# gitAugust/Aruco_Slam

Hardware: AMD Instinct MI355X
Metric: frames/s (detect+pose+EKF) at 1280x720, 20 markers, 200 landmarks (higher is better)
Workload: dtype u8/f64; 1 GPU; cfg2: 1280x720 gray stream per GPU, 20 markers/frame in view, 200-landmark EKF (N=603), frames resident in HBM, detector {'polygonalApproxAccuracyRate': 0.03, 'doCornerRefinement': 1}; streams=1, ekf=True, asserted=every frame: 20 markers detected, 20 corrections fused, map_gather=none

## Files before the change

aruco_slam_amd/csrc/detect.hip:

```cpp
#include "common.h"
#include "detect.h"
#include <cfloat>
#include <climits>
#include <cstdlib>
#include <algorithm>

namespace aslam {

__device__ __forceinline__ int dir_dx(int s) { return (int)((0x901Au >> (2 * s)) & 3u) - 1; }
__device__ __forceinline__ int dir_dy(int s) { return (int)((0xA901u >> (2 * s)) & 3u) - 1; }
__device__ __forceinline__ int first_outer(unsigned m) { return (m & 1u) ? 0 : (m & 128u) ? 7 : (m & 64u) ? 6 : 5; }
__device__ __forceinline__ int first_hole(unsigned m) { return 31 - __clz((int)(m & 0xFEu)); }


__device__ __forceinline__ unsigned byte_is_zero(unsigned x) { return ~(((x & 0x7F7F7F7Fu) + 0x7F7F7F7Fu) | x) & 0x80808080u; }

constexpr int TW = 64, TH = 32, HALO = 12;
constexpr int LW = TW + 2 * HALO;
constexpr int LH = TH + 2 * HALO;
constexpr int kBlockStarts = 1024;

template <int R> __device__ __forceinline__ bool box_is_fg(const unsigned (*I)[LW + 1], int ly, int lx, int v_plus_c) {
    constexpr int k2 = (2 * R + 1) * (2 * R + 1);
    const int sum = (int)(I[ly + R + 1][lx + R + 1] - I[ly - R][lx + R + 1] - I[ly + R + 1][lx - R] + I[ly - R][lx - R]);
    return 2 * sum >= k2 * (2 * v_plus_c - 1);
}
__device__ __forceinline__ bool box_is_fg_r(const unsigned (*I)[LW + 1], int ly, int lx, int R, int v_plus_c) {
    const int k2 = (2 * R + 1) * (2 * R + 1);
    const int sum = (int)(I[ly + R + 1][lx + R + 1] - I[ly - R][lx + R + 1] - I[ly + R + 1][lx - R] + I[ly - R][lx - R]);
    return 2 * sum >= k2 * (2 * v_plus_c - 1);
}

#ifdef ASLAM_THR_STAMPS
#define THR_STAMP(i) do { if (tid == 0 && blockIdx.x == 4000) tst[i] = clock64(); } while (0)
#else
#define THR_STAMP(i) do { } while (0)
#endif
template <bool kDefaultWindows>
__global__ __launch_bounds__(256) void k_threshold(const uint8_t* __restrict__ in, int channels, size_t in_frame_stride,
                                                   size_t in_row_step, uint8_t* __restrict__ gray_out,
                                                   uint8_t* __restrict__ nbr, DetectCfg cfg,
                                                   unsigned* __restrict__ starts, unsigned* __restrict__ n_starts,
                                                   unsigned* __restrict__ nodeplane, Counters* ctr, int nframes) {
    __shared__ uint8_t g[LH][LW + 4];
    __shared__ unsigned I[LH + 1][LW + 1];
    __shared__ unsigned long long sRow[kScales][TH + 2];
    __shared__ unsigned long long sRing[kScales][2];
    __shared__ unsigned sLutRow[3][64];
    __shared__ unsigned sStart[kBlockStarts];
    __shared__ unsigned sNStart, sBase;

    const int tid = threadIdx.x;
    const int rows = cfg.rows, cols = cfg.cols;
    const unsigned gx = (unsigned)(cols + TW - 1) / TW, gy = (unsigned)(rows + TH - 1) / TH;
    const unsigned per_xcd = gridDim.x >> 3;
    const unsigned logical = (blockIdx.x & 7u) * per_xcd + (blockIdx.x >> 3);
    if (logical >= gx * gy * (unsigned)nframes) return;
    const int b = (int)(logical / (gx * gy));
    const unsigned rem = logical - (unsigned)b * gx * gy;
    const int x0 = (int)(rem % gx) * TW, y0 = (int)(rem / gx) * TH;
    const uint8_t* src = in + (size_t)b * in_frame_stride;
#ifdef ASLAM_THR_STAMPS
    long long tst[8] = {0};
#endif
    if (tid == 0) sNStart = 0;
    THR_STAMP(0);

    if (channels == 1 && (in_row_step & 3) == 0 && ((size_t)src & 3) == 0) {
        constexpr int kPasses = (LH * (LW / 4) + 255) / 256;
        unsigned v[kPasses];
#pragma unroll
        for (int p = 0; p < kPasses; p++) {
            const int i = tid + 256 * p;
            v[p] = 0;
            if (i < LH * (LW / 4)) {
                const int ly = i / (LW / 4), q = i - ly * (LW / 4);
                const int gy = min(max(y0 + ly - HALO, 0), rows - 1);
                const int gx = x0 + 4 * q - HALO;
                const uint8_t* rowp = src + (size_t)gy * in_row_step;
                if (gx >= 0 && gx + 3 < cols) {
                    v[p] = *reinterpret_cast<const unsigned*>(rowp + gx);
                } else {
                    for (int k = 0; k < 4; k++) v[p] |= (unsigned)rowp[min(max(gx + k, 0), cols - 1)] << (8 * k);
                }
            }
        }
#pragma unroll
        for (int p = 0; p < kPasses; p++) {
            const int i = tid + 256 * p;
            if (i < LH * (LW / 4)) {
                const int ly = i / (LW / 4), q = i - ly * (LW / 4);
                *reinterpret_cast<unsigned*>(&g[ly][4 * q]) = v[p];
            }
        }
    } else {
        for (int i = tid; i < LH * LW; i += 256) {
            int ly = i / LW, lx = i - ly * LW;
            int gx = min(max(x0 + lx - HALO, 0), cols - 1);
            int gy = min(max(y0 + ly - HALO, 0), rows - 1);
            const uint8_t* p = src + (size_t)gy * in_row_step + (size_t)gx * channels;
            unsigned v;
            if (channels == 3) v = (p[0] * 1868u + p[1] * 9617u + p[2] * 4899u + 8192u) >> 14;
            else v = p[0];
            g[ly][lx] = (uint8_t)v;
        }
    }
    __syncthreads();
    THR_STAMP(1);

    if (gray_out != nullptr) {
        for (int i = tid; i < TH * TW; i += 256) {
            int ty = i / TW, tx = i - ty * TW;
            int gx = x0 + tx, gy = y0 + ty;
            if (gx < cols && gy < rows) gray_out[((size_t)b * rows + gy) * cols + gx] = g[ty + HALO][tx + HALO];
        }
    }

    {
        const int q = tid >> 6, r = tid & 63;
        if (r < LH) {
            unsigned s = 0;
            for (int k = 0; k < LW / 4; k++) { s += g[r][q * (LW / 4) + k]; I[r + 1][q * (LW / 4) + k + 1] = s; }
        }
        if (tid < LW + 1) I[0][tid] = 0;
        if (tid < LH) I[tid + 1][0] = 0;
        __syncthreads();
        unsigned add = 0;
        if (r < LH)
            for (int qq = 0; qq < q; qq++) add += I[r + 1][(qq + 1) * (LW / 4)];
        __syncthreads();
        if (r < LH && q > 0)
            for (int k = 0; k < LW / 4; k++) I[r + 1][q * (LW / 4) + k + 1] += add;
    }
    __syncthreads();
    {
        const int h = tid >> 7, c = tid & 127;
        if (c < LW) {
            unsigned s = 0;
            for (int k = 0; k < LH / 2; k++) { s += I[h * (LH / 2) + k + 1][c + 1]; I[h * (LH / 2) + k + 1][c + 1] = s; }
        }
        __syncthreads();
        if (c < LW && h == 1) {
            const unsigned add = I[LH / 2][c + 1];
            for (int k = 0; k < LH / 2; k++) I[LH / 2 + k + 1][c + 1] += add;
        }
    }
    __syncthreads();
    THR_STAMP(2);

    auto thr_bits = [&](int by, int bx) -> unsigned {
        const int gx = x0 + bx - 1, gy = y0 + by - 1;
        unsigned bits = 0;
        if (gx >= 0 && gx < cols && gy >= 0 && gy < rows) {
            const int lx = bx - 1 + HALO, ly = by - 1 + HALO;
            const int vc = (int)g[ly][lx] + cfg.thresh_c;
            if (kDefaultWindows) {
                if (box_is_fg<1>(I, ly, lx, vc)) bits |= 1u;
                if (box_is_fg<6>(I, ly, lx, vc)) bits |= 2u;
                if (box_is_fg<11>(I, ly, lx, vc)) bits |= 4u;
            } else {
#pragma unroll
                for (int s = 0; s < kScales; s++)
                    if (s < cfg.n_scales && box_is_fg_r(I, ly, lx, cfg.win_r[s], vc)) bits |= 1u << s;
            }
        }
        return bits;
    };
    {
        const int wave = tid >> 6, lane = tid & 63;
        for (int by = wave; by < TH + 2; by += 4) {
            const unsigned bits = thr_bits(by, lane);
#pragma unroll
            for (int s = 0; s < kScales; s++) {
                const unsigned long long row = __ballot((bits >> s) & 1u);
                if (lane == 0) sRow[s][by] = row;
            }
        }
        if (wave < 2) {
            const unsigned bits = lane < TH + 2 ? thr_bits(lane, TW + wave) : 0u;
#pragma unroll
            for (int s = 0; s < kScales; s++) {
                const unsigned long long col = __ballot((bits >> s) & 1u);
                if (lane == 0) sRing[s][wave] = col;
            }
        }
        if (tid < 3 * 64) {
            const unsigned r = tid >> 6, v = tid & 63u;
            unsigned w = 0;
            for (unsigned j = 0; j < 4; j++) {
                const unsigned a = (v >> j) & 1u, b = (v >> (j + 1)) & 1u, c = (v >> (j + 2)) & 1u;
                const unsigned m = r == 0 ? (c << 1) | (b << 2) | (a << 3) : r == 1 ? c | (a << 4) : (a << 5) | (b << 6) | (c << 7);
                w |= m << (8 * j);
            }
            sLutRow[r][v] = w;
        }
    }
    __syncthreads();
    THR_STAMP(3);

    for (int u = tid; u < TH * TW / 4; u += 256) {
        const int ty = u / (TW / 4), tx4 = (u - ty * (TW / 4)) * 4;
        const int gy = y0 + ty;
        const bool row_on_grid = (gy & cfg.cut_mask) == 0;
        const unsigned grid4 = row_on_grid ? 15u : ((tx4 & cfg.cut_mask) == 0 ? 1u : 0u);
        unsigned out[kScales] = {0, 0, 0};
        unsigned emit = 0;
#pragma unroll
        for (int s = 0; s < kScales; s++) {
            unsigned six[3];
#pragma unroll
            for (int r = 0; r < 3; r++) {
                const int by = ty + r;
                unsigned v = (unsigned)(sRow[s][by] >> tx4) & 63u;
                if (tx4 == TW - 4) v |= ((unsigned)(sRing[s][0] >> by) & 1u) << 4 | ((unsigned)(sRing[s][1] >> by) & 1u) << 5;
                six[r] = v;
            }
            const unsigned m4 = sLutRow[0][six[0]] | sLutRow[1][six[1]] | sLutRow[2][six[2]];
            out[s] = m4;
            const unsigned fgb = (((six[1] >> 1) & 15u) * 0x00204081u & 0x01010101u) << 7;
            const unsigned hole_x = (m4 & 0x03030303u) ^ 0x02020202u;
            const unsigned cand = fgb & ((byte_is_zero(m4 & 0x1E1E1E1Eu) & ~byte_is_zero(m4)) | byte_is_zero(hole_x));
            emit |= (((cand >> 7) | (cand >> 14) | (cand >> 21) | (cand >> 28)) & 15u) << (4 * s);
            emit |= (((six[1] >> 1) & grid4) & 15u) << (4 * s);
        }
        for (unsigned rest = emit; rest; rest &= rest - 1u) {
            const int bit = __ffs((int)rest) - 1, s = bit >> 2, j = bit & 3;
            const unsigned gx = (unsigned)(x0 + tx4 + j);
            const unsigned m = (out[s] >> (8 * j)) & 0xFFu;
            const bool outer = m != 0 && (m & 0x1Eu) == 0, hole = (m & 3u) == 2u;
            const unsigned s0 = outer ? (unsigned)first_outer(m) : (unsigned)first_hole(m);
            unsigned cut = 0;
            if (row_on_grid || (gx & (unsigned)cfg.cut_mask) == 0) cut = m & ~((m >> 1) | (m << 7)) & 0xFFu;
            if (outer || hole) cut &= ~(1u << s0);
            const unsigned cnt = (unsigned)__popc(cut) + ((outer || hole) ? 1u : 0u);
            if (cnt == 0) continue;
            const unsigned k = atomicAdd(&sNStart, cnt);
            const bool staged = k + cnt <= (unsigned)kBlockStarts;
            unsigned kk = 0;
            bool fits = true;
            if (!staged) {
                for (unsigned e = k; e < (unsigned)kBlockStarts; e++) sStart[e] = kNone;
                kk = atomicAdd(&n_starts[b], cnt);
                fits = kk + cnt <= cfg.cap_starts;
                if (fits) nodeplane[((size_t)b * kScales + s) * nbr_plane_bytes(rows, cfg.pitch) + nbr_index((int)gx, gy, cfg.pitch)] = kk;
                else atomicOr(&ctr->overflow, (unsigned)kOvfStarts);
            }
            unsigned e = 0;
            auto put = [&](unsigned v) {
                if (staged) sStart[k + e] = v;
                else if (fits) starts[(size_t)b * cfg.cap_starts + kk + e] = v;
                e++;
            };
            if (outer || hole) put(pack_node(gx, (unsigned)gy, s0, (unsigned)s, outer ? kNodeOuter : kNodeHole));
            for (unsigned c2 = cut; c2; c2 &= c2 - 1u) put(pack_node(gx, (unsigned)gy, (unsigned)(__ffs((int)c2) - 1), (unsigned)s, kNodeCut));
        }
        if (gy < rows) {
#pragma unroll
            for (int s = 0; s < kScales; s++) {
                unsigned* dst = reinterpret_cast<unsigned*>(nbr + ((size_t)b * kScales + s) * nbr_plane_bytes(rows, cfg.pitch) +
                                                            nbr_index(x0 + tx4, gy, cfg.pitch));
                *dst = out[s];
            }
        }
    }
    __syncthreads();
    THR_STAMP(4);
    const unsigned ns = min(sNStart, (unsigned)kBlockStarts);
    if (tid == 0 && ns > 0) sBase = atomicAdd(&n_starts[b], ns);
    __syncthreads();
    for (unsigned i = tid; i < ns; i += 256) {
        const unsigned k = sBase + i, e = sStart[i];
        if (k < cfg.cap_starts) {
            starts[(size_t)b * cfg.cap_starts + k] = e;
            if (e != kNone && (i == 0 || ((sStart[i - 1] ^ e) & kNodePixelMask) != 0))
                nodeplane[((size_t)b * kScales + ((e >> 27) & 3u)) * nbr_plane_bytes(rows, cfg.pitch) +
                          nbr_index((int)(e & 0xFFFu), (int)((e >> 12) & 0xFFFu), cfg.pitch)] = k;
        } else {
            atomicOr(&ctr->overflow, (unsigned)kOvfStarts);
        }
    }
#ifdef ASLAM_THR_STAMPS
    THR_STAMP(5);
    if (tid == 0 && blockIdx.x == 4000) printf("thr tile: load %lld integral %lld threshold %lld masks %lld flush %lld\n", tst[1] - tst[0], tst[2] - tst[1], tst[3] - tst[2], tst[4] - tst[3], tst[5] - tst[4]);
#endif
}

__global__ __launch_bounds__(256) void k_clear_counts(int nframes, Counters* ctr, unsigned* a0, unsigned* a1, unsigned* a2, unsigned* a3, unsigned* a4) {
    const int i = blockIdx.x * 256 + threadIdx.x;
    if (i < kCounterHeads) reinterpret_cast<unsigned*>(ctr)[i] = 0u;
    if (i < nframes) { a0[i] = 0u; a1[i] = 0u; a2[i] = 0u; a3[i] = 0u; a4[i] = 0u; }
}

__global__ __launch_bounds__(256) void k_prefix(int nframes, const unsigned* __restrict__ counts, unsigned cap, unsigned per_ticket,
                                                unsigned* __restrict__ pre ) {
    __shared__ unsigned sPart[256];
    const int tid = threadIdx.x;
    const int per = (nframes + 255) / 256;
    unsigned s = 0;
    for (int k = 0; k < per; k++) {
        int f = tid * per + k;
        if (f < nframes) s += (min(counts[f], cap) + per_ticket - 1) / per_ticket;
    }
    sPart[tid] = s;
    __syncthreads();
    if (tid == 0) {
        unsigned acc = 0;
        for (int i = 0; i < 256; i++) { unsigned v = sPart[i]; sPart[i] = acc; acc += v; }
        pre[nframes] = acc;
    }
    __syncthreads();
    unsigned acc = sPart[tid];
    for (int k = 0; k < per; k++) {
        int f = tid * per + k;
        if (f < nframes) { pre[f] = acc; acc += (min(counts[f], cap) + per_ticket - 1) / per_ticket; }
    }
}

__device__ __forceinline__ int ticket_frame(const unsigned* sPre, int nframes, unsigned ticket) {
    int lo = 0, hi = nframes;
    while (hi - lo > 1) {
        int mid = (lo + hi) >> 1;
        if (sPre[mid] <= ticket) lo = mid; else hi = mid;
    }
    return lo;
}

constexpr int kMaxFramesPerCall = 1024;

__device__ __forceinline__ void load_ticket_ranges(unsigned* sPre, const unsigned* __restrict__ pre, const unsigned* __restrict__ counts,
                                                   unsigned cap, int nframes, int tid, int nthreads) {
    if (nframes == 1) {
        if (tid == 0) { sPre[0] = 0u; sPre[1] = min(counts[0], cap); }
    } else {
        for (int i = tid; i <= nframes; i += nthreads) sPre[i] = pre[i];
    }
}

struct Walk {
    int x, y, s;
};
__device__ __forceinline__ void walk_step(Walk& w, unsigned m) {
    unsigned r = ((m | (m << 8)) >> (w.s + 1)) & 0xFFu;
    int k = __ffs((int)r) - 1;
    int s2 = (w.s + 1 + k) & 7;
    w.x += dir_dx(s2);
    w.y += dir_dy(s2);
    w.s = (s2 + 4) & 7;
}

constexpr int kTraceChunk = 64;
constexpr int kSegRepsBusy = 32, kSegRepsRefill = 8;


__device__ __forceinline__ void build_step_table(unsigned short* sStep, int tid, int nthreads) {
    for (int i = tid; i < 256 * 8; i += nthreads) {
        const unsigned m = (unsigned)i >> 3;
        const int sd = i & 7;
        Walk t{0, 0, sd};
        if (m != 0) walk_step(t, m);
        const bool co = m != 0 && (m & 0x1Eu) == 0 && sd == first_outer(m);
        const bool ch = (m & 3u) == 2u && sd == first_hole(m);
        const bool cut = ((m >> sd) & 1u) != 0 && ((m >> ((sd + 1) & 7)) & 1u) == 0;
        sStep[i] = (unsigned short)((unsigned)(t.x + 1) | ((unsigned)(t.y + 1) << 2) | ((unsigned)t.s << 4) | (co ? 0x80u : 0u) | (ch ? 0x100u : 0u) |
                                    (cut ? 0x200u : 0u));
    }
}
__device__ __forceinline__ bool on_cut_grid(int x, int y, int mask) { return ((x & mask) == 0) || ((y & mask) == 0); }

__global__ __launch_bounds__(64) void k_seg(const uint8_t* __restrict__ nbr, DetectCfg cfg, int nframes,
                                            const unsigned* __restrict__ starts, const unsigned* __restrict__ n_starts,
                                            const unsigned* __restrict__ nodeplane,
                                            const unsigned* __restrict__ pre, Counters* ctr,
                                            NodeRec* __restrict__ nodes) {
    __shared__ unsigned sPre[kMaxFramesPerCall + 1];
    __shared__ unsigned short sStep[256 * 8];
    const int lane = threadIdx.x & 63;
    build_step_table(sStep, lane, 64);
    load_ticket_ranges(sPre, pre, n_starts, cfg.cap_starts, nframes, lane, 64);
    __syncthreads();
    const unsigned total = sPre[nframes];
    const int pitch = cfg.pitch;
    const size_t plane_bytes = nbr_plane_bytes(cfg.rows, pitch);

    int mode = 0;
    bool drained = false;
    unsigned lo = 0, hi = 0;
    const uint8_t* plane = nbr;
    const unsigned* idplane = nodeplane;
    Walk w{0, 0, 0};
    int n = 0, f = 0, area = 0;
    unsigned self = 0, state0 = 0;

    for (;;) {
        const unsigned long long idle = __ballot(mode == 0);
        if (idle != 0ull && !drained) {
            if (lo == hi) {
                unsigned base = 0;
                if (lane == 0) base = atomicAdd(&ctr->q_trace, (unsigned)kTraceChunk);
                base = __shfl(base, 0);
                lo = base;
                hi = min(base + (unsigned)kTraceChunk, total);
                if (lo >= total) { drained = true; lo = hi = 0; }
            }
            const unsigned take = min((unsigned)__popcll(idle), hi - lo);
            const unsigned rank = (unsigned)__popcll(idle & ((1ull << lane) - 1ull));
            if (mode == 0 && rank < take) {
                const unsigned ticket = lo + rank;
                if (!(ticket >= sPre[f] && ticket < sPre[f + 1])) f = ticket_frame(sPre, nframes, ticket);
                self = ticket - sPre[f];
                const unsigned e = starts[(size_t)f * cfg.cap_starts + self];
                const unsigned type = (e >> 29) & 3u;
                if (type == kNodeInvalid) {
                    nodes[(size_t)f * cfg.cap_starts + self] = NodeRec{kNone, kNone, 0u, 0};
                } else {
                    const int x = (int)(e & 0xFFFu), y = (int)((e >> 12) & 0xFFFu);
                    const unsigned sc = (e >> 27) & 3u;
                    plane = nbr + ((size_t)f * kScales + sc) * plane_bytes;
                    idplane = nodeplane + ((size_t)f * kScales + sc) * plane_bytes;
                    state0 = e;
                    w = Walk{x, y, (int)((e >> 24) & 7u)};
                    area = 0;
                    n = 0;
                    mode = 1;
                }
            }
            lo += take;
        }
        if (__ballot(mode != 0) == 0ull) {
            if (drained) break;
            continue;
        }
        const int reps = (idle == 0ull || drained) ? kSegRepsBusy : kSegRepsRefill;
        for (int rep = 0; rep < reps; rep++) {
            if (mode == 1) {
                const unsigned m = plane[nbr_index(w.x, w.y, pitch)];
                const unsigned st = sStep[(m << 3) | (unsigned)w.s];
                const bool arrived = n > 0 && ((st & 0x180u) != 0 || ((st & 0x200u) != 0 && on_cut_grid(w.x, w.y, cfg.cut_mask)));
                if (arrived) {
                    const unsigned want = pack_node((unsigned)w.x, (unsigned)w.y, (unsigned)w.s, (state0 >> 27) & 3u, 0u);
                    const unsigned cnt = min(n_starts[f], cfg.cap_starts);
                    unsigned id = idplane[nbr_index(w.x, w.y, pitch)];
                    unsigned found = kNone;
                    for (int t = 0; t < 9 && id < cnt; t++, id++) {
                        const unsigned e2 = starts[(size_t)f * cfg.cap_starts + id];
                        if (((e2 ^ want) & kNodePixelMask) != 0) break;
                        if (((e2 ^ want) & kNodeStateMask) == 0) { found = id; break; }
                    }
                    nodes[(size_t)f * cfg.cap_starts + self] = NodeRec{state0, found, (unsigned)n, area};
                    mode = 0;
                } else {
                    const int ddx = (int)(st & 3u) - 1, ddy = (int)((st >> 2) & 3u) - 1;
                    area += w.x * ddy - ddx * w.y;
                    w.x += ddx; w.y += ddy; w.s = (int)((st >> 4) & 7u);
                    n++;
                    if (n > cfg.max_perim) {
                        nodes[(size_t)f * cfg.cap_starts + self] = NodeRec{state0, kNone, (unsigned)n, area};
                            mode = 0;
                    }
                }
            }
            if (__ballot(mode != 0) == 0ull) break;
        }
    }
}

__device__ __forceinline__ int node_key(unsigned state, int cols) {
    return (int)((state >> 12) & 0xFFFu) * cols + (int)(state & 0xFFFu) + (((state >> 29) & 3u) == kNodeHole ? 1 : 0);
}
__device__ __forceinline__ void void_tickets(WriteRec* wl, unsigned wbase, unsigned wcap, unsigned cap_write) {
    for (unsigned long long t = wbase; t < (unsigned long long)wbase + wcap && t < cap_write; t++) wl[t] = WriteRec{0u, kNone, 0u, 0u};
}
constexpr int kLinkThreads = 1024;
constexpr unsigned kLinkLdsNodes = 32000;
constexpr unsigned kLinkSlots = 1536;
struct LinkSlot {
    int a;
    int b;
    int c;
    unsigned d;
};
__global__ __launch_bounds__(kLinkThreads) void k_link(DetectCfg cfg, const unsigned* __restrict__ n_starts, Counters* ctr,
                                                       const NodeRec* __restrict__ nodes, unsigned lds_nodes, unsigned* __restrict__ link_todo,
                                                       ContourRec* __restrict__ contours, unsigned* __restrict__ n_contours,
                                                       unsigned* __restrict__ n_points, WriteRec* __restrict__ wlist, unsigned* __restrict__ n_write) {
    ASLAM_DYN_LDS(dyn_lds);
    __shared__ unsigned sNSlots, sActive;
    const int tid = threadIdx.x;
    const int f = blockIdx.x;
    const int cols = cfg.cols;
    const unsigned nn = min(n_starts[f], cfg.cap_starts);
    const NodeRec* gn = nodes + (size_t)f * cfg.cap_starts;
    if (nn > lds_nodes) {
        if (tid == 0) link_todo[f] = 1u;
        return;
    }
    unsigned* sPair = reinterpret_cast<unsigned*>(dyn_lds);
    LinkSlot* sSlot = reinterpret_cast<LinkSlot*>(sPair + lds_nodes);
    unsigned* sIsLeader = reinterpret_cast<unsigned*>(sSlot + kLinkSlots);
    if (tid == 0) { sNSlots = 0; sActive = 0; }
    for (unsigned i = tid; i < (nn + 31u) / 32u; i += kLinkThreads) sIsLeader[i] = 0u;

    for (unsigned i = tid; i < nn; i += kLinkThreads) {
        const NodeRec r = gn[i];
        const bool dead = r.state == kNone || r.nxt == kNone || r.nxt >= nn;
        sPair[i] = dead ? (0u | (i << 16)) : ((i + 1u) | (r.nxt << 16));
    }
    __syncthreads();
    int rounds = 1;
    while ((1u << rounds) < nn) rounds++;
    for (int r = 0; r <= rounds; r++) {
        for (unsigned i = tid; i < nn; i += kLinkThreads) {
            const unsigned w = sPair[i], wp = sPair[w >> 16];
            sPair[i] = min(w & 0xFFFFu, wp & 0xFFFFu) | (wp & 0xFFFF0000u);
        }
        __syncthreads();
    }
    for (unsigned i = tid; i < nn; i += kLinkThreads) {
        const unsigned lead = sPair[i] & 0xFFFFu;
        unsigned w = 0xFFFF0000u;
        if (lead != 0u) {
            const NodeRec r = gn[i];
            w = min(r.len, 0xFFFFu) | (r.nxt << 16);
            if (lead == i + 1u) atomicOr(&sIsLeader[i >> 5], 1u << (i & 31u));
        }
        sPair[i] = w;
    }
    __syncthreads();
    for (int r = 0; r <= rounds + 1; r++) {
        bool active = false;
        for (unsigned i = tid; i < nn; i += kLinkThreads) {
            const unsigned w = sPair[i], p = w >> 16;
            if (p >= 0x8000u || ((sIsLeader[p >> 5] >> (p & 31u)) & 1u)) continue;
            const unsigned wp = sPair[p];
            sPair[i] = min((w & 0xFFFFu) + (wp & 0xFFFFu), 0xFFFFu) | (wp & 0xFFFF0000u);
            active = true;
        }
        if (active) sActive = (unsigned)r + 1u;
        __syncthreads();
        const bool any = sActive == (unsigned)r + 1u;
        __syncthreads();
        if (!any) break;
    }
    for (unsigned i = tid; i < nn; i += kLinkThreads) {
        if (!((sIsLeader[i >> 5] >> (i & 31u)) & 1u)) continue;
        const unsigned w = sPair[i], n = w & 0xFFFFu;
        unsigned v = 0x7FFFu;
        if ((int)n >= cfg.min_perim && (int)n <= cfg.max_perim && (w >> 16) == i) {
            const unsigned slot = atomicAdd(&sNSlots, 1u);
            if (slot < kLinkSlots) {
                sSlot[slot] = LinkSlot{0, INT_MAX, INT_MAX, n};
                v = slot;
            }
        }
        sPair[i] = n | ((0x8000u | v) << 16);
    }
    __syncthreads();
    if (sNSlots > kLinkSlots) {
        if (tid == 0) link_todo[f] = 1u;
        return;
    }
    if (tid == 0) link_todo[f] = 0u;
    auto slot_of = [&](unsigned i) -> int {
        unsigned w = sPair[i];
        if (!(w >> 31)) w = sPair[w >> 16];
        const unsigned v = (w >> 16) & 0x7FFFu;
        return (w >> 31) && v != 0x7FFFu ? (int)v : -1;
    };
    for (unsigned i = tid; i < nn; i += kLinkThreads) {
        const int sl = slot_of(i);
        if (sl < 0) continue;
        const NodeRec r = gn[i];
        atomicAdd(&sSlot[sl].a, r.area);
        const unsigned type = (r.state >> 29) & 3u;
        if (type == kNodeOuter) atomicMin(&sSlot[sl].b, node_key(r.state, cols));
        if (type == kNodeHole) atomicMin(&sSlot[sl].c, node_key(r.state, cols));
    }
    __syncthreads();
    for (unsigned i = tid; i < nn; i += kLinkThreads) {
        if (!((sIsLeader[i >> 5] >> (i & 31u)) & 1u)) continue;
        const unsigned v = (sPair[i] >> 16) & 0x7FFFu;
        if (v == 0x7FFFu) continue;
        LinkSlot& s = sSlot[v];
        const bool is_hole = s.a > 0;
        const int ckey = is_hole ? s.c : s.b;
        s.b = ckey == INT_MAX ? -1 : (int)((unsigned)ckey | (is_hole ? 0x80000000u : 0u));
        s.a = (int)kNone;
// ... 761 lines not shown
```

Measured before the change: 57280 frames/s.

## Specialize threshold kernel for interior tiles and process two rows per thread

Adds an interior-tile fast path that loads the tile with incremental pointer stepping and skips per-pixel bounds checks in the adaptive-threshold bit-row pass. The bit-row pass is restructured so each wave handles contiguous rows and the right-edge ring columns are packed into the same shared array. The LUT build is hoisted before the load. The mask/emit stage now handles two rows per thread, reusing four bit rows for two outputs. This removes the old strided loop and cuts shared-memory reads and index math. In exchange it adds register pressure and more complex emit decoding, and the nbr store addressing now assumes a particular layout (offset 8*r for the next row).

```diff
diff --git a/aruco_slam_amd/csrc/detect.hip b/aruco_slam_amd/csrc/detect.hip
--- a/aruco_slam_amd/csrc/detect.hip
+++ b/aruco_slam_amd/csrc/detect.hip
@@ -30,9 +30,65 @@
     const int sum = (int)(I[ly + R + 1][lx + R + 1] - I[ly - R][lx + R + 1] - I[ly + R + 1][lx - R] + I[ly - R][lx - R]);
     return 2 * sum >= k2 * (2 * v_plus_c - 1);
 }
+template <bool kDefaultWindows>
+__device__ __forceinline__ void thr_px(const uint8_t (*g)[LW + 4], const unsigned (*I)[LW + 1], const DetectCfg& cfg, int ly, int lx, bool (&fg)[kScales]) {
+    const int vc = (int)g[ly][lx] + min(max(cfg.thresh_c, -256), 256);
+    if (kDefaultWindows) {
+        fg[0] = box_is_fg<1>(I, ly, lx, vc);
+        fg[1] = box_is_fg<6>(I, ly, lx, vc);
+        fg[2] = box_is_fg<11>(I, ly, lx, vc);
+    } else {
+#pragma unroll
+        for (int s = 0; s < kScales; s++) fg[s] = s < cfg.n_scales && box_is_fg_r(I, ly, lx, cfg.win_r[s], vc);
+    }
+}
+
+constexpr int kRingRows = TH + 2, kRowsPerWave = (kRingRows + 3) / 4;
+template <bool kDefaultWindows, bool kInterior>
+__device__ __forceinline__ void thr_bit_rows(const uint8_t (*g)[LW + 4], const unsigned (*I)[LW + 1], unsigned (*sRow)[kRingRows][4],
+                                             const DetectCfg& cfg, int x0, int y0, int tid) {
+    const int wave = tid >> 6, lane = tid & 63;
+    const int by0 = min(kRowsPerWave * wave, kRingRows - (kRowsPerWave - 1));
+    const int nby = wave < 2 ? kRowsPerWave : kRowsPerWave - 1;
+    const bool col_ok = kInterior || (x0 + lane - 1 >= 0 && x0 + lane - 1 < cfg.cols);
+#pragma unroll
+    for (int i = 0; i < kRowsPerWave; i++) {
+        if (i < nby) {
+            const int by = by0 + i;
+            bool fg[kScales];
+            thr_px<kDefaultWindows>(g, I, cfg, by - 1 + HALO, lane - 1 + HALO, fg);
+            const bool ok = kInterior || (col_ok && y0 + by - 1 >= 0 && y0 + by - 1 < cfg.rows);
+            unsigned long long row[kScales];
+#pragma unroll
+            for (int s = 0; s < kScales; s++) row[s] = __ballot(fg[s] && ok);
+            if (lane == 0) {
+#pragma unroll
+                for (int s = 0; s < kScales; s++) { sRow[s][by][0] = (unsigned)row[s]; sRow[s][by][1] = (unsigned)(row[s] >> 32); }
+            }
+        }
+    }
+    if (wave == 3) {
+        const int by = min(lane, kRingRows - 1);
+        const bool row_ok = kInterior || (y0 + by - 1 >= 0 && y0 + by - 1 < cfg.rows);
+        unsigned w[kScales] = {0, 0, 0};
+#pragma unroll
+        for (int k = 0; k < 2; k++) {
+            bool fg[kScales];
+            thr_px<kDefaultWindows>(g, I, cfg, by - 1 + HALO, TW + k - 1 + HALO, fg);
+            const bool ok = kInterior || (row_ok && x0 + TW + k - 1 < cfg.cols);
+#pragma unroll
+            for (int s = 0; s < kScales; s++) w[s] |= (fg[s] && ok) ? 1u << k : 0u;
+        }
+        if (lane < kRingRows) {
+#pragma unroll
+            for (int s = 0; s < kScales; s++) sRow[s][lane][2] = w[s];
+        }
+    }
+}
 
 #ifdef ASLAM_THR_STAMPS
-#define THR_STAMP(i) do { if (tid == 0 && blockIdx.x == 4000) tst[i] = clock64(); } while (0)
+#define THR_STAMP_BLOCK 4008
+#define THR_STAMP(i) do { if (tid == 0 && blockIdx.x == THR_STAMP_BLOCK) tst[i] = clock64(); } while (0)
 #else
 #define THR_STAMP(i) do { } while (0)
 #endif
@@ -44,8 +100,7 @@
                                                    unsigned* __restrict__ nodeplane, Counters* ctr, int nframes) {
     __shared__ uint8_t g[LH][LW + 4];
     __shared__ unsigned I[LH + 1][LW + 1];
-    __shared__ unsigned long long sRow[kScales][TH + 2];
-    __shared__ unsigned long long sRing[kScales][2];
+    __shared__ unsigned sRow[kScales][kRingRows][4];
     __shared__ unsigned sLutRow[3][64];
     __shared__ unsigned sStart[kBlockStarts];
     __shared__ unsigned sNStart, sBase;
@@ -64,33 +119,66 @@
     long long tst[8] = {0};
 #endif
     if (tid == 0) sNStart = 0;
+    const bool interior = x0 >= HALO && x0 + TW + HALO <= cols && y0 >= HALO && y0 + TH + HALO <= rows;
     THR_STAMP(0);
+    if (tid < 3 * 64) {
+        const unsigned r = tid >> 6, v = tid & 63u;
+        unsigned w = 0;
+        for (unsigned j = 0; j < 4; j++) {
+            const unsigned a = (v >> j) & 1u, b = (v >> (j + 1)) & 1u, c = (v >> (j + 2)) & 1u;
+            const unsigned m = r == 0 ? (c << 1) | (b << 2) | (a << 3) : r == 1 ? c | (a << 4) : (a << 5) | (b << 6) | (c << 7);
+            w |= m << (8 * j);
+        }
+        sLutRow[r][v] = w;
+    }
 
     if (channels == 1 && (in_row_step & 3) == 0 && ((size_t)src & 3) == 0) {
-        constexpr int kPasses = (LH * (LW / 4) + 255) / 256;
+        constexpr int kRowDwords = LW / 4, kDwords = LH * kRowDwords;
+        constexpr int kPasses = (kDwords + 255) / 256;
         unsigned v[kPasses];
-#pragma unroll
-        for (int p = 0; p < kPasses; p++) {
-            const int i = tid + 256 * p;
-            v[p] = 0;
-            if (i < LH * (LW / 4)) {
-                const int ly = i / (LW / 4), q = i - ly * (LW / 4);
-                const int gy = min(max(y0 + ly - HALO, 0), rows - 1);
-                const int gx = x0 + 4 * q - HALO;
-                const uint8_t* rowp = src + (size_t)gy * in_row_step;
-                if (gx >= 0 && gx + 3 < cols) {
-                    v[p] = *reinterpret_cast<const unsigned*>(rowp + gx);
-                } else {
-                    for (int k = 0; k < 4; k++) v[p] |= (unsigned)rowp[min(max(gx + k, 0), cols - 1)] << (8 * k);
-                }
-            }
-        }
-#pragma unroll
-        for (int p = 0; p < kPasses; p++) {
-            const int i = tid + 256 * p;
-            if (i < LH * (LW / 4)) {
-                const int ly = i / (LW / 4), q = i - ly * (LW / 4);
-                *reinterpret_cast<unsigned*>(&g[ly][4 * q]) = v[p];
+        if (interior) {
+            constexpr int kStepRows = 256 / kRowDwords, kStepQ = 256 - kStepRows * kRowDwords;
+            int ly = tid / kRowDwords, q = tid - ly * kRowDwords;
+            const uint8_t* p = src + (size_t)(y0 - HALO + ly) * in_row_step + (size_t)(x0 - HALO + 4 * q);
+            const size_t step_same = (size_t)kStepRows * in_row_step + 4 * kStepQ;
+            const size_t step_wrap = (size_t)(kStepRows + 1) * in_row_step - 4 * (kRowDwords - kStepQ);
+            int off[kPasses];
+#pragma unroll
+            for (int k = 0; k < kPasses; k++) {
+                off[k] = ly * (LW + 4) + 4 * q;
+                v[k] = (k < kPasses - 1 || tid < kDwords - 256 * (kPasses - 1)) ? *reinterpret_cast<const unsigned*>(p) : 0u;
+                const bool wrap = q + kStepQ >= kRowDwords;
+                p += wrap ? step_wrap : step_same;
+                ly += wrap ? kStepRows + 1 : kStepRows;
+                q += wrap ? kStepQ - kRowDwords : kStepQ;
+            }
+#pragma unroll
+            for (int k = 0; k < kPasses; k++)
+                if (k < kPasses - 1 || tid < kDwords - 256 * (kPasses - 1)) *reinterpret_cast<unsigned*>(&g[0][0] + off[k]) = v[k];
+        } else {
+#pragma unroll
+            for (int p = 0; p < kPasses; p++) {
+                const int i = tid + 256 * p;
+                v[p] = 0;
+                if (i < kDwords) {
+                    const int ly = i / kRowDwords, q = i - ly * kRowDwords;
+                    const int gy = min(max(y0 + ly - HALO, 0), rows - 1);
+                    const int gx = x0 + 4 * q - HALO;
+                    const uint8_t* rowp = src + (size_t)gy * in_row_step;
+                    if (gx >= 0 && gx + 3 < cols) {
+                        v[p] = *reinterpret_cast<const unsigned*>(rowp + gx);
+                    } else {
+                        for (int k = 0; k < 4; k++) v[p] |= (unsigned)rowp[min(max(gx + k, 0), cols - 1)] << (8 * k);
+                    }
+                }
+            }
+#pragma unroll
+            for (int p = 0; p < kPasses; p++) {
+                const int i = tid + 256 * p;
+                if (i < kDwords) {
+                    const int ly = i / kRowDwords, q = i - ly * kRowDwords;
+                    *reinterpret_cast<unsigned*>(&g[ly][4 * q]) = v[p];
+                }
             }
         }
     } else {
@@ -148,85 +236,45 @@
     __syncthreads();
     THR_STAMP(2);
 
-    auto thr_bits = [&](int by, int bx) -> unsigned {
-        const int gx = x0 + bx - 1, gy = y0 + by - 1;
-        unsigned bits = 0;
-        if (gx >= 0 && gx < cols && gy >= 0 && gy < rows) {
-            const int lx = bx - 1 + HALO, ly = by - 1 + HALO;
-            const int vc = (int)g[ly][lx] + cfg.thresh_c;
-            if (kDefaultWindows) {
-                if (box_is_fg<1>(I, ly, lx, vc)) bits |= 1u;
-                if (box_is_fg<6>(I, ly, lx, vc)) bits |= 2u;
-                if (box_is_fg<11>(I, ly, lx, vc)) bits |= 4u;
-            } else {
-#pragma unroll
-                for (int s = 0; s < kScales; s++)
-                    if (s < cfg.n_scales && box_is_fg_r(I, ly, lx, cfg.win_r[s], vc)) bits |= 1u << s;
-            }
-        }
-        return bits;
-    };
+    if (interior) thr_bit_rows<kDefaultWindows, true>(g, I, sRow, cfg, x0, y0, tid);
+    else thr_bit_rows<kDefaultWindows, false>(g, I, sRow, cfg, x0, y0, tid);
+    __syncthreads();
+    THR_STAMP(3);
+
     {
-        const int wave = tid >> 6, lane = tid & 63;
-        for (int by = wave; by < TH + 2; by += 4) {
-            const unsigned bits = thr_bits(by, lane);
-#pragma unroll
-            for (int s = 0; s < kScales; s++) {
-                const unsigned long long row = __ballot((bits >> s) & 1u);
-                if (lane == 0) sRow[s][by] = row;
-            }
-        }
-        if (wave < 2) {
-            const unsigned bits = lane < TH + 2 ? thr_bits(lane, TW + wave) : 0u;
-#pragma unroll
-            for (int s = 0; s < kScales; s++) {
-                const unsigned long long col = __ballot((bits >> s) & 1u);
-                if (lane == 0) sRing[s][wave] = col;
-            }
-        }
-        if (tid < 3 * 64) {
-            const unsigned r = tid >> 6, v = tid & 63u;
-            unsigned w = 0;
-            for (unsigned j = 0; j < 4; j++) {
-                const unsigned a = (v >> j) & 1u, b = (v >> (j + 1)) & 1u, c = (v >> (j + 2)) & 1u;
-                const unsigned m = r == 0 ? (c << 1) | (b << 2) | (a << 3) : r == 1 ? c | (a << 4) : (a << 5) | (b << 6) | (c << 7);
-                w |= m << (8 * j);
-            }
-            sLutRow[r][v] = w;
-        }
-    }
-    __syncthreads();
-    THR_STAMP(3);
-
-    for (int u = tid; u < TH * TW / 4; u += 256) {
-        const int ty = u / (TW / 4), tx4 = (u - ty * (TW / 4)) * 4;
-        const int gy = y0 + ty;
-        const bool row_on_grid = (gy & cfg.cut_mask) == 0;
-        const unsigned grid4 = row_on_grid ? 15u : ((tx4 & cfg.cut_mask) == 0 ? 1u : 0u);
-        unsigned out[kScales] = {0, 0, 0};
+        const int ty = (tid >> 4) * 2, tx4 = (tid & 15) * 4;
+        const int gy0 = y0 + ty;
+        const int kw = tx4 >> 5, sh = tx4 & 31;
+        const unsigned col_grid = (tx4 & cfg.cut_mask) == 0 ? 1u : 0u;
+        const unsigned grid4[2] = {(gy0 & cfg.cut_mask) == 0 ? 15u : col_grid, ((gy0 + 1) & cfg.cut_mask) == 0 ? 15u : col_grid};
+        unsigned out[2][kScales];
         unsigned emit = 0;
 #pragma unroll
         for (int s = 0; s < kScales; s++) {
-            unsigned six[3];
-#pragma unroll
-            for (int r = 0; r < 3; r++) {
-                const int by = ty + r;
-                unsigned v = (unsigned)(sRow[s][by] >> tx4) & 63u;
-                if (tx4 == TW - 4) v |= ((unsigned)(sRing[s][0] >> by) & 1u) << 4 | ((unsigned)(sRing[s][1] >> by) & 1u) << 5;
-                six[r] = v;
-            }
-            const unsigned m4 = sLutRow[0][six[0]] | sLutRow[1][six[1]] | sLutRow[2][six[2]];
-            out[s] = m4;
-            const unsigned fgb = (((six[1] >> 1) & 15u) * 0x00204081u & 0x01010101u) << 7;
-            const unsigned hole_x = (m4 & 0x03030303u) ^ 0x02020202u;
-            const unsigned cand = fgb & ((byte_is_zero(m4 & 0x1E1E1E1Eu) & ~byte_is_zero(m4)) | byte_is_zero(hole_x));
-            emit |= (((cand >> 7) | (cand >> 14) | (cand >> 21) | (cand >> 28)) & 15u) << (4 * s);
-            emit |= (((six[1] >> 1) & grid4) & 15u) << (4 * s);
+            unsigned six[4];
+#pragma unroll
+            for (int r = 0; r < 4; r++) {
+                const unsigned* w = &sRow[s][ty + r][kw];
+                six[r] = (unsigned)((((unsigned long long)w[1] << 32) | w[0]) >> sh) & 63u;
+            }
+#pragma unroll
+            for (int r = 0; r < 2; r++) {
+                const unsigned m4 = sLutRow[0][six[r]] | sLutRow[1][six[r + 1]] | sLutRow[2][six[r + 2]];
+                out[r][s] = m4;
+                const unsigned fgb = (((six[r + 1] >> 1) & 15u) * 0x00204081u & 0x01010101u) << 7;
+                const unsigned hole_x = (m4 & 0x03030303u) ^ 0x02020202u;
+                const unsigned cand = fgb & ((byte_is_zero(m4 & 0x1E1E1E1Eu) & ~byte_is_zero(m4)) | byte_is_zero(hole_x));
+                emit |= (((cand >> 7) | (cand >> 14) | (cand >> 21) | (cand >> 28)) & 15u) << (12 * r + 4 * s);
+                emit |= (((six[r + 1] >> 1) & grid4[r]) & 15u) << (12 * r + 4 * s);
+            }
         }
         for (unsigned rest = emit; rest; rest &= rest - 1u) {
-            const int bit = __ffs((int)rest) - 1, s = bit >> 2, j = bit & 3;
+            const int bit = __ffs((int)rest) - 1, r = bit >= 12 ? 1 : 0, s = (bit - 12 * r) >> 2, j = bit & 3;
+            const int gy = gy0 + r;
+            const bool row_on_grid = (gy & cfg.cut_mask) == 0;
             const unsigned gx = (unsigned)(x0 + tx4 + j);
-            const unsigned m = (out[s] >> (8 * j)) & 0xFFu;
+            const unsigned o0 = s == 0 ? out[0][0] : s == 1 ? out[0][1] : out[0][2], o1 = s == 0 ? out[1][0] : s == 1 ? out[1][1] : out[1][2];
+            const unsigned m = ((r ? o1 : o0) >> (8 * j)) & 0xFFu;
             const bool outer = m != 0 && (m & 0x1Eu) == 0, hole = (m & 3u) == 2u;
             const unsigned s0 = outer ? (unsigned)first_outer(m) : (unsigned)first_hole(m);
             unsigned cut = 0;
@@ -254,12 +302,13 @@
             if (outer || hole) put(pack_node(gx, (unsigned)gy, s0, (unsigned)s, outer ? kNodeOuter : kNodeHole));
             for (unsigned c2 = cut; c2; c2 &= c2 - 1u) put(pack_node(gx, (unsigned)gy, (unsigned)(__ffs((int)c2) - 1), (unsigned)s, kNodeCut));
         }
-        if (gy < rows) {
-#pragma unroll
-            for (int s = 0; s < kScales; s++) {
-                unsigned* dst = reinterpret_cast<unsigned*>(nbr + ((size_t)b * kScales + s) * nbr_plane_bytes(rows, cfg.pitch) +
-                                                            nbr_index(x0 + tx4, gy, cfg.pitch));
-                *dst = out[s];
+        const size_t plane = nbr_plane_bytes(rows, cfg.pitch);
+        uint8_t* dst = nbr + (size_t)b * kScales * plane + nbr_index(x0 + tx4, gy0, cfg.pitch);
+#pragma unroll
+        for (int r = 0; r < 2; r++) {
+            if (gy0 + r < rows) {
+#pragma unroll
+                for (int s = 0; s < kScales; s++) *reinterpret_cast<unsigned*>(dst + s * plane + 8 * r) = out[r][s];
             }
         }
     }
@@ -281,7 +330,7 @@
     }
 #ifdef ASLAM_THR_STAMPS
     THR_STAMP(5);
-    if (tid == 0 && blockIdx.x == 4000) printf("thr tile: load %lld integral %lld threshold %lld masks %lld flush %lld\n", tst[1] - tst[0], tst[2] - tst[1], tst[3] - tst[2], tst[4] - tst[3], tst[5] - tst[4]);
+    if (tid == 0 && blockIdx.x == THR_STAMP_BLOCK) printf("thr tile: load %lld integral %lld threshold %lld masks %lld flush %lld\n", tst[1] - tst[0], tst[2] - tst[1], tst[3] - tst[2], tst[4] - tst[3], tst[5] - tst[4]);
 #endif
 }
 
```

Result: no change. 57030 frames/s (-0.4%).
